# rubund/gnuais

Measured on AMD Instinct MI355X. Metric: Msamples/s demodulated (N-channel batch, full chain), higher is better.
Workload: dtype f32 FIR on int16 samples; u32 PLL/HDLC/CRC; 1 GPU; C3: 16384 ch x 48000 samples @48 kHz per GPU, full chain incl. HDLC/CRC-16; channels_per_gpu=16384, samples_per_channel=48000, parallelism=channels sharded over 1 GPU(s), one process per GPU, no collectives

## Files before the change

gnuais_amd/csrc/pll_common.h:

```cpp
#pragma once
#include <hip/hip_runtime.h>
#include <stdint.h>

#include "kernels.h"

namespace gnuais {

__device__ __forceinline__ uint32_t wave_max(uint32_t v)
{
#pragma unroll
    for (int o = 32; o; o >>= 1) {
        const uint32_t u = (uint32_t) __shfl_xor((int) v, o);
        v = u > v ? u : v;
    }
    return v;
}

constexpr int PLL_PACKW = PACK_STRIDE + 1;
constexpr int PLL_LUT_BYTES = 2048;

__device__ __forceinline__ void lds_flag_store(uint32_t *f, uint32_t v)
{
    asm volatile("" ::: "memory");
    __hip_atomic_store(f, v, __ATOMIC_RELAXED, __HIP_MEMORY_SCOPE_WORKGROUP);
    asm volatile("" ::: "memory");
}
__device__ __forceinline__ uint32_t lds_flag_load(uint32_t *f)
{
    asm volatile("" ::: "memory");
    const uint32_t v = __hip_atomic_load(f, __ATOMIC_RELAXED, __HIP_MEMORY_SCOPE_WORKGROUP);
    asm volatile("" ::: "memory");
    return v;
}

__host__ __device__ inline int n_seg_cap(int L)
{
    return (((L + 31) >> 5) + SEG_WORDS - 1) / SEG_WORDS;
}

__device__ __forceinline__ void pll_fill_lut(uint64_t *lut, int tid, int n_threads)
{
    for (int v = tid; v < 256; v += n_threads) {
        uint64_t e = 0;
        int n = 0;
        for (int b = 7; b >= 0; --b)
            if (v & (1 << b)) e |= (uint64_t) (7 - b) << (8 * n++);
        lut[v] = e;
    }
}

}
```

gnuais_amd/csrc/pll_h3.hip:

```cpp
#include <hip/hip_runtime.h>
#include <stdint.h>

#include <algorithm>
#include "kernels.h"
#include "pll_common.h"

namespace gnuais {

constexpr int H3_BLK = 128;
constexpr int H3_WORDS = H3_BLK / 32;
constexpr int H3_STRIP = H3_BLK + 12;
constexpr int H3_SEG_BLKS = SEG_LEN / H3_BLK;
constexpr int H3_NH = 3;
constexpr int H3_SLOTS = 2 * H3_NH;
constexpr int H3_NPACK = 4;
constexpr int H3_OFF_CNT = 64 * H3_STRIP, H3_OFF_NG = H3_OFF_CNT + 256;
constexpr int H3_SLOT_BYTES = H3_OFF_NG + 64;
constexpr int H3_FLAG_WORDS = 32 + 2 * 64 + 4 * 64;
constexpr int H3_NEED_LDS = PLL_LUT_BYTES + H3_SLOTS * H3_SLOT_BYTES + H3_NPACK * PLL_PACKW * 64 * 4 + H3_FLAG_WORDS * 4;
static_assert((H3_STRIP / 4) % 2 == 1 && H3_STRIP % 4 == 0, "odd dword stride: lanes hit different banks");
static_assert(SEG_LEN % H3_BLK == 0 && H3_NEED_LDS <= PLL_LDS_BYTES, "segments are whole blocks; the stage's LDS share");

enum { F_RDONE = 1, F_SEGPUB = 2, F_WRITTEN = 3, F_LAST = 4, F_SCAN = 8  };


__device__ __forceinline__ void h3_expand_block(const uint32_t (&S)[H3_WORDS], uint32_t &prev, int nv, uint8_t *lds,
                                                uint8_t *slot, const uint64_t *lut, int lane)
{
    uint32_t cur = (uint32_t) (slot - lds) + (uint32_t) (lane * H3_STRIP);
    const uint32_t cur0 = cur;
#pragma unroll
    for (int w = 0; w < H3_WORDS; ++w) {
        const int k = nv - 32 * w;
        uint32_t d = S[w] ^ ((S[w] >> 1) | (prev << 31));
        if (k <= 0) {
            d = 0;
        } else if (k < 32) {
            d &= ~0u << (32 - k);
            prev = (S[w] >> (32 - k)) & 1u;
        } else {
            prev = S[w] & 1u;
        }
        uint64_t ent[4];
#pragma unroll
        for (int y = 0; y < 4; ++y)
            ent[y] = lut[(d >> (24 - 8 * y)) & 0xffu];
#pragma unroll
        for (int y = 0; y < 4; ++y) {
            const uint32_t base = 0x01010101u * (uint32_t) (32 * w + 8 * y);
            const uint64_t e = ent[y] + (((uint64_t) base << 32) | base);
            asm volatile("ds_write_b64 %0, %1" :: "v"(cur), "v"(e) : "memory");
            cur += (uint32_t) __popc((d >> (24 - 8 * y)) & 0xffu);
        }
    }
    const uint32_t cnt = cur - cur0;
    reinterpret_cast<uint32_t *>(slot + H3_OFF_CNT)[lane] = cnt;
    const uint32_t ng = wave_max((cnt + 3u) >> 2);
    if (lane == 0) reinterpret_cast<uint32_t *>(slot + H3_OFF_NG)[0] = ng;
}

#define H3_STEP(k, E, kk)                                                                 \
    "v_cmpx_lt_i32 vcc, " #kk ", %[rem]\n\t"                                              \
    "v_mul_u32_u24_sdwa %[T], %[K8], %[" #E "] dst_sel:DWORD dst_unused:UNUSED_PAD src0_sel:DWORD src1_sel:BYTE_" #k "\n\t" \
    "v_add_u32 %[U], %[X], %[T]\n\t"                                                      \
    "v_bfe_i32 %[um], %[U], 23, 1\n\t"                                                    \
    "v_xad_u32 %[X], %[Q], %[um], %[X]\n\t"                                               \
    "v_lshlrev_b32_sdwa %[T], %[U], %[one] dst_sel:DWORD dst_unused:UNUSED_PAD src0_sel:BYTE_3 src1_sel:DWORD\n\t" \
    "v_xor_b32 %[M], %[M], %[T]\n\t"

__device__ __forceinline__ uint32_t h3_rows(uint32_t &X, uint32_t cnt, uint32_t ad, uint32_t ng, uint32_t Q, uint32_t K8)
{
    uint32_t U, um, T, E, F, G, H, M = 0, one = 1;
    int32_t rem = (int32_t) cnt;
    uint32_t np = (ng + 1u) >> 1;
    unsigned long long sv;
    asm volatile(
        "s_mov_b64 %[sv], exec\n\t"
        "ds_read_b32 %[E], %[ad]\n\t"
        "ds_read_b32 %[F], %[ad] offset:4\n\t"
        "1:\n\t"
        "ds_read_b32 %[G], %[ad] offset:8\n\t"
        "ds_read_b32 %[H], %[ad] offset:12\n\t"
        "s_waitcnt lgkmcnt(2)\n\t"
        "v_or_b32 %[X], 0xff, %[X]\n\t"
        H3_STEP(0, E, 0) H3_STEP(1, E, 1) H3_STEP(2, E, 2) H3_STEP(3, E, 3)
        "v_or_b32 %[X], 0xff, %[X]\n\t"
        H3_STEP(0, F, 4) H3_STEP(1, F, 5) H3_STEP(2, F, 6) H3_STEP(3, F, 7)
        "s_sub_u32 %[np], %[np], 1\n\t"
        "s_cmp_eq_u32 %[np], 0\n\t"
        "s_cbranch_scc1 2f\n\t"
        "ds_read_b32 %[E], %[ad] offset:16\n\t"
        "ds_read_b32 %[F], %[ad] offset:20\n\t"
        "s_waitcnt lgkmcnt(2)\n\t"
        "v_or_b32 %[X], 0xff, %[X]\n\t"
        H3_STEP(0, G, 8) H3_STEP(1, G, 9) H3_STEP(2, G, 10) H3_STEP(3, G, 11)
        "v_or_b32 %[X], 0xff, %[X]\n\t"
        H3_STEP(0, H, 12) H3_STEP(1, H, 13) H3_STEP(2, H, 14) H3_STEP(3, H, 15)
        "v_add_u32 %[ad], 16, %[ad]\n\t"
        "v_subrev_u32 %[rem], 16, %[rem]\n\t"
        "s_sub_u32 %[np], %[np], 1\n\t"
        "s_cmp_lg_u32 %[np], 0\n\t"
        "s_cbranch_scc1 1b\n\t"
        "2:\n\t"
        "s_mov_b64 exec, %[sv]\n\t"
        "s_waitcnt lgkmcnt(0)\n\t"
        : [X] "+v"(X), [U] "=&v"(U), [um] "=&v"(um), [T] "=&v"(T), [E] "=&v"(E), [F] "=&v"(F), [G] "=&v"(G), [H] "=&v"(H),
          [M] "+v"(M), [ad] "+v"(ad), [rem] "+v"(rem), [np] "+s"(np), [sv] "=&s"(sv)
        : [Q] "s"(Q), [K8] "v"(K8), [one] "v"(one)
        : "vcc", "scc", "memory");
    return M;
}

__device__ __forceinline__ uint32_t h3_write_pack(uint32_t *pk, uint32_t nb, uint32_t par, bool live,
                                                  uint32_t *__restrict__ dst, uint32_t *__restrict__ dcnt)
{
    uint32_t pd = 0;
#pragma unroll 1
    for (int g = 0; g < PACK_STRIDE / 4; ++g) {
        uint32_t o[4];
#pragma unroll
        for (int j = 0; j < 4; ++j) {
            const int w = 4 * g + j;
            const uint32_t tg = pk[w * 64];
            pk[w * 64] = 0;
            const int k = (int) nb - 32 * w;
            o[j] = ~tg & (k >= 32 ? ~0u : k > 0 ? (1u << k) - 1u : 0u);
            if (k >= 0 && k < 32) pd = (tg >> k) & 1u;
        }
        if (g == 0 && nb) o[0] ^= par;
        if (live) reinterpret_cast<uint4 *>(dst)[g] = make_uint4(o[0], o[1], o[2], o[3]);
    }
    if (live) *dcnt = nb;
    return nb ? pd : (par ^ pd);
}

__global__ __launch_bounds__(64 * (1 + H3_NH)) __attribute__((amdgpu_waves_per_eu(4, 8))) void pll_h3_kernel(
    const uint4 *__restrict__ sgn4, uint32_t *__restrict__ pllst, uint32_t *__restrict__ prevst,
    uint32_t *__restrict__ lastbit, uint32_t *__restrict__ segbits, uint32_t *__restrict__ segcnt,
    uint32_t *__restrict__ watchdog, int N, int L, int n_seg_alloc, uint32_t pllinc)
{
    extern __shared__ uint8_t lds[];
    uint64_t *lut = reinterpret_cast<uint64_t *>(lds);
    uint8_t *slots = lds + PLL_LUT_BYTES;
    uint32_t *pack = reinterpret_cast<uint32_t *>(slots + H3_SLOTS * H3_SLOT_BYTES);
    uint32_t *flag = pack + H3_NPACK * PLL_PACKW * 64;
    uint32_t *sign0 = flag + 32, *sign1 = flag + 32 + 64;
    uint32_t *nbuf = flag + 32 + 128;
    const int lane = threadIdx.x & 63, role = threadIdx.x >> 6;
    const int cg = blockIdx.x * 64 + lane;
    const int c = cg < N ? cg : N - 1;
    const bool live = cg < N;
    const int n_seg = n_seg_cap(L);
    const int n_blk = (L + H3_BLK - 1) / H3_BLK;
    if (threadIdx.x < 32) flag[threadIdx.x] = (threadIdx.x >= F_SCAN && threadIdx.x < F_SCAN + H3_NH) ? threadIdx.x - F_SCAN : 0u;
    if (role == 0) sign0[lane] = prevst[c] & 1u;
    pll_fill_lut(lut, (int) threadIdx.x, 64 * (1 + H3_NH));
    for (int q = threadIdx.x; q < H3_NPACK * PLL_PACKW * 64; q += 64 * (1 + H3_NH)) pack[q] = 0;
    __syncthreads();
    const unsigned long long t_start = wall_clock64();
    auto expired = [=]() {
        if (wall_clock64() - t_start <= 20000000ull) return false;
        if (lane == 0) atomicOr(watchdog, 1u);
        return true;
    };
#define peek(f) __builtin_amdgcn_readfirstlane((int) lds_flag_load(flag + (f)))
    __builtin_amdgcn_s_setprio(3);

    if (role >= 1) {
        const int h = role - 1;
        const uint4 *__restrict__ src = sgn4 + c;
        uint32_t par = h == 0 ? (lastbit[c] ^ sign0[lane]) & 1u : 0u;
        int wseg = 0;
#define H3_LOAD_BLOCK(b)                                   \
    do {                                                                                                        \
        const int bb = (b) < n_blk ? (b) : 0;                                                                   \
        q = src[(size_t) bb * (size_t) N];                                                                      \
        pw = reinterpret_cast<const uint32_t *>(src + (size_t) (bb > 0 ? bb - 1 : 0) * (size_t) N)[3];          \
    } while (0)
        uint4 q;
        uint32_t pw;
        H3_LOAD_BLOCK(h);
        bool dead = false;
        for (int bs = h; !dead; bs += H3_NH) {
            if (bs >= n_blk && !(h == 0 && wseg < n_seg)) break;
            if (h == 0) {
                while (wseg < n_seg && peek(F_SEGPUB) >= wseg + 1) {
                    uint32_t *pk = pack + (wseg & (H3_NPACK - 1)) * PLL_PACKW * 64 + lane;
                    const uint32_t nb = nbuf[(wseg & 3) * 64 + lane];
                    par = h3_write_pack(pk, nb, par, live, segbits + ((size_t) cg * n_seg_alloc + wseg) * PACK_STRIDE,
                                        segcnt + (size_t) cg * n_seg_alloc + wseg);
                    lds_flag_store(flag + F_WRITTEN, (uint32_t) (++wseg));
                }
                if (bs >= n_blk) {
                    if (expired()) dead = true;
                    __builtin_amdgcn_s_sleep(4);
                    continue;
                }
            }
            while (peek(F_RDONE) < bs - (H3_SLOTS - 1) && !dead) {
                if (expired()) dead = true;
                __builtin_amdgcn_s_sleep(8);
            }
            if (dead) break;
            {
                uint32_t S[H3_WORDS] = {q.x, q.y, q.z, q.w};
                uint32_t prev = bs == 0 ? sign0[lane] : (pw & 1u);
                H3_LOAD_BLOCK(bs + H3_NH);
                h3_expand_block(S, prev, L - bs * H3_BLK, lds, slots + (bs % H3_SLOTS) * H3_SLOT_BYTES, lut, lane);
                lds_flag_store(flag + F_SCAN + h, (uint32_t) (bs + H3_NH));
                if (bs == n_blk - 1) {
                    sign1[lane] = prev;
                    lds_flag_store(flag + F_LAST, 1u);
                    if (live) prevst[cg] = prev;
                }
            }
        }
        if (h == 0) {
            while (lds_flag_load(flag + F_LAST) == 0 && !dead)
                if (expired()) dead = true;
            if (live && !dead) {
                for (int s = n_seg; s < n_seg_alloc; ++s) segcnt[(size_t) cg * n_seg_alloc + s] = 0;
                lastbit[cg] = (sign1[lane] ^ par) & 1u;
            }
        }
        return;
    }

    uint32_t X = ((pllst[c] & 0xffffu) << 8) | 0xffu;
    const uint32_t Q = (uint32_t) __builtin_amdgcn_readfirstlane((int) ((pllinc / 16u) << 8));
    const uint32_t K8 = pllinc << 8;
    bool dead = false;
    for (int s = 0; s < n_seg && !dead; ++s) {
        while (peek(F_WRITTEN) < s - (H3_NPACK - 1) && !dead) {
            if (expired()) dead = true;
            __builtin_amdgcn_s_sleep(2);
        }
        uint32_t segbase = 0;
        uint32_t *pk = pack + (s & (H3_NPACK - 1)) * PLL_PACKW * 64 + lane;
        const int b1 = (s + 1) * H3_SEG_BLKS < n_blk ? (s + 1) * H3_SEG_BLKS : n_blk;
        for (int b = s * H3_SEG_BLKS; b < b1 && !dead; ++b) {
            const uint8_t *slot = slots + (b % H3_SLOTS) * H3_SLOT_BYTES;
            uint32_t cnt, ng;
            for (;;) {
                uint32_t f, g;
                asm volatile("ds_read_b32 %0, %3\n\tds_read_b32 %1, %4\n\tds_read_b32 %2, %5\n\ts_waitcnt lgkmcnt(0)"
                             : "=&v"(f), "=&v"(cnt), "=&v"(g)
                             : "v"((uint32_t) (reinterpret_cast<uint8_t *>(flag + F_SCAN + b % H3_NH) - lds)),
                               "v"((uint32_t) (slot + H3_OFF_CNT - lds) + (uint32_t) lane * 4u),
                               "v"((uint32_t) (slot + H3_OFF_NG - lds))
                             : "memory");
                ng = (uint32_t) __builtin_amdgcn_readfirstlane((int) g);
                if (__builtin_amdgcn_readfirstlane((int) f) >= b + 1) break;
                if (expired()) { dead = true; break; }
                __builtin_amdgcn_s_sleep(1);
            }
            if (dead) break;
            segbase += X >> 24;
            X &= 0x00ffffffu;
            if (ng) {
                const uint32_t M = h3_rows(X, cnt, (uint32_t) (slot - lds) + (uint32_t) (lane * H3_STRIP), ng, Q, K8);
                lds_flag_store(flag + F_RDONE, (uint32_t) (b + 1));
                const uint32_t sh = segbase & 31u, w = segbase >> 5;
                atomicXor(pk + w * 64, M << sh);
                atomicXor(pk + w * 64 + 64, (M >> 1) >> (31u - sh));
            } else {
                lds_flag_store(flag + F_RDONE, (uint32_t) (b + 1));
            }
            const int blen = L - b * H3_BLK < H3_BLK ? L - b * H3_BLK : H3_BLK;
            X += (uint32_t) blen * K8;
        }
        if (dead) break;
        X |= 0xffu;
        nbuf[(s & 3) * 64 + lane] = segbase + (X >> 24);
        X = (X & 0x00ffff00u) | 0xffu;
        lds_flag_store(flag + F_SEGPUB, (uint32_t) (s + 1));
    }
    if (live && !dead) pllst[cg] = (X >> 8) & 0xffffu;
}

int pll_need_lds() { return H3_NEED_LDS; }

hipError_t pll_prepare_device()
{
    return hipFuncSetAttribute((const void *) pll_h3_kernel, hipFuncAttributeMaxDynamicSharedMemorySize, 160 * 1024);
}

int pll_form_of(const PllLaunch &a)
{
    if ((a.variant == 7 || (a.variant == 0 && a.N <= PLL_TP_MAX_CHANNELS)) && pll_tp_applicable(a)) return 7;
    return 8;
}

hipError_t launch_pll(const PllLaunch &a, hipStream_t stream)
{
    if (pll_form_of(a) == 7) return launch_pll_tp(a, stream);
    const int n_cu = a.n_cu > 0 ? a.n_cu : 256;
    const int groups = (a.N + 63) / 64, per_cu = (groups + n_cu - 1) / n_cu;
    const int lds = per_cu <= 1 ? std::max(H3_NEED_LDS, PLL_LDS_BYTES) : std::max(H3_NEED_LDS, (160 * 1024 / per_cu) & ~1023);
    if (lds > 160 * 1024) return hipErrorInvalidValue;
    hipLaunchKernelGGL(pll_h3_kernel, dim3(groups), dim3(64 * (1 + H3_NH)), lds, stream, (const uint4 *) a.sgn, a.pll, a.prev, a.lastbit,
                       a.segbits, a.segcnt, a.watchdog, a.N, a.L, a.n_seg, a.pllinc);
    return hipGetLastError();
}

}
```

Baseline: 1.646 million Msamples/s.

## Streamline H3 block expansion: alignbit transitions, SDWA LUT addressing, DPP max, pointer-stepped loads

Reworks the H3 transition-expansion producer. Full blocks now compute transitions with alignbit, and the partial-bit masking is kept only for the tail block. LUT addresses are formed directly with SDWA byte-select shifts, and the wave-wide max uses a DPP reduction that leaves the result in lane 63 instead of shuffle-xor. Block loads use incrementally stepped pointers with a readfirstlane'd scalar block index, and the row consumer handles odd group counts by entering the unrolled loop mid-way. The goal is fewer VALU and address instructions in the producer wave. The risks are reliance on the LUT sitting at LDS offset 0 and on the DPP row semantics being correct.

```diff
diff --git a/gnuais_amd/csrc/pll_common.h b/gnuais_amd/csrc/pll_common.h
--- a/gnuais_amd/csrc/pll_common.h
+++ b/gnuais_amd/csrc/pll_common.h
@@ -13,6 +13,20 @@
         const uint32_t u = (uint32_t) __shfl_xor((int) v, o);
         v = u > v ? u : v;
     }
+    return v;
+}
+
+__device__ __forceinline__ uint32_t wave_max_in_lane63(uint32_t v)
+{
+#define PLL_DPP_MAX(ctrl, rows) \
+    { const uint32_t u = (uint32_t) __builtin_amdgcn_update_dpp(0, (int) v, ctrl, rows, 0xf, false); v = u > v ? u : v; }
+    PLL_DPP_MAX(0x111, 0xf)
+    PLL_DPP_MAX(0x112, 0xf)
+    PLL_DPP_MAX(0x114, 0xf)
+    PLL_DPP_MAX(0x118, 0xf)
+    PLL_DPP_MAX(0x142, 0xa)
+    PLL_DPP_MAX(0x143, 0xc)
+#undef PLL_DPP_MAX
     return v;
 }
 
diff --git a/gnuais_amd/csrc/pll_h3.hip b/gnuais_amd/csrc/pll_h3.hip
--- a/gnuais_amd/csrc/pll_h3.hip
+++ b/gnuais_amd/csrc/pll_h3.hip
@@ -24,39 +24,62 @@
 enum { F_RDONE = 1, F_SEGPUB = 2, F_WRITTEN = 3, F_LAST = 4, F_SCAN = 8  };
 
 
-__device__ __forceinline__ void h3_expand_block(const uint32_t (&S)[H3_WORDS], uint32_t &prev, int nv, uint8_t *lds,
-                                                uint8_t *slot, const uint64_t *lut, int lane)
-{
-    uint32_t cur = (uint32_t) (slot - lds) + (uint32_t) (lane * H3_STRIP);
-    const uint32_t cur0 = cur;
+__device__ __forceinline__ void h3_expand_block(const uint32_t (&d)[H3_WORDS], uint8_t *lds, uint8_t *slot, int lane)
+{
+    const uint32_t cur0 = (uint32_t) (slot - lds) + (uint32_t) (lane * H3_STRIP);
+    uint32_t cur = cur0;
+    const uint32_t three = 3;
+#pragma unroll
+    for (int w = 0; w < H3_WORDS; ++w) {
+        uint32_t a[4], at[4];
+        asm("v_lshlrev_b32_sdwa %0, %1, %2 dst_sel:DWORD dst_unused:UNUSED_PAD src0_sel:DWORD src1_sel:BYTE_3" : "=v"(a[0]) : "v"(three), "v"(d[w]));
+        asm("v_lshlrev_b32_sdwa %0, %1, %2 dst_sel:DWORD dst_unused:UNUSED_PAD src0_sel:DWORD src1_sel:BYTE_2" : "=v"(a[1]) : "v"(three), "v"(d[w]));
+        asm("v_lshlrev_b32_sdwa %0, %1, %2 dst_sel:DWORD dst_unused:UNUSED_PAD src0_sel:DWORD src1_sel:BYTE_1" : "=v"(a[2]) : "v"(three), "v"(d[w]));
+        asm("v_lshlrev_b32_sdwa %0, %1, %2 dst_sel:DWORD dst_unused:UNUSED_PAD src0_sel:DWORD src1_sel:BYTE_0" : "=v"(a[3]) : "v"(three), "v"(d[w]));
+        uint64_t ent[4];
+#pragma unroll
+        for (int y = 0; y < 4; ++y)
+            ent[y] = *(const __attribute__((address_space(3))) uint64_t *) (uintptr_t) a[y];
+#pragma unroll
+        for (int y = 0; y < 4; ++y) {
+            at[y] = cur;
+            cur += (uint32_t) __popc(a[y]);
+        }
+#pragma unroll
+        for (int y = 0; y < 4; ++y) {
+            const uint32_t base = 0x01010101u * (uint32_t) (32 * w + 8 * y);
+            const uint64_t e = ent[y] + (((uint64_t) base << 32) | base);
+            asm volatile("ds_write_b64 %0, %1" :: "v"(at[y]), "v"(e) : "memory");
+        }
+    }
+    const uint32_t cnt = cur - cur0;
+    reinterpret_cast<uint32_t *>(slot + H3_OFF_CNT)[lane] = cnt;
+    const uint32_t ng = wave_max_in_lane63((cnt + 3u) >> 2);
+    if (lane == 63) reinterpret_cast<uint32_t *>(slot + H3_OFF_NG)[0] = ng;
+}
+
+__device__ __forceinline__ void h3_transitions_full(const uint32_t (&S)[H3_WORDS], uint32_t pw, uint32_t (&d)[H3_WORDS])
+{
+#pragma unroll
+    for (int w = 0; w < H3_WORDS; ++w)
+        d[w] = S[w] ^ __builtin_amdgcn_alignbit(w ? S[w - 1] : pw, S[w], 1);
+}
+
+__device__ __forceinline__ void h3_transitions_tail(const uint32_t (&S)[H3_WORDS], uint32_t &prev, int nv, uint32_t (&d)[H3_WORDS])
+{
 #pragma unroll
     for (int w = 0; w < H3_WORDS; ++w) {
         const int k = nv - 32 * w;
-        uint32_t d = S[w] ^ ((S[w] >> 1) | (prev << 31));
+        d[w] = S[w] ^ ((S[w] >> 1) | (prev << 31));
         if (k <= 0) {
-            d = 0;
+            d[w] = 0;
         } else if (k < 32) {
-            d &= ~0u << (32 - k);
+            d[w] &= ~0u << (32 - k);
             prev = (S[w] >> (32 - k)) & 1u;
         } else {
             prev = S[w] & 1u;
         }
-        uint64_t ent[4];
-#pragma unroll
-        for (int y = 0; y < 4; ++y)
-            ent[y] = lut[(d >> (24 - 8 * y)) & 0xffu];
-#pragma unroll
-        for (int y = 0; y < 4; ++y) {
-            const uint32_t base = 0x01010101u * (uint32_t) (32 * w + 8 * y);
-            const uint64_t e = ent[y] + (((uint64_t) base << 32) | base);
-            asm volatile("ds_write_b64 %0, %1" :: "v"(cur), "v"(e) : "memory");
-            cur += (uint32_t) __popc((d >> (24 - 8 * y)) & 0xffu);
-        }
-    }
-    const uint32_t cnt = cur - cur0;
-    reinterpret_cast<uint32_t *>(slot + H3_OFF_CNT)[lane] = cnt;
-    const uint32_t ng = wave_max((cnt + 3u) >> 2);
-    if (lane == 0) reinterpret_cast<uint32_t *>(slot + H3_OFF_NG)[0] = ng;
+    }
 }
 
 #define H3_STEP(k, E, kk)                                                                 \
@@ -76,6 +99,16 @@
     unsigned long long sv;
     asm volatile(
         "s_mov_b64 %[sv], exec\n\t"
+        "s_bitcmp0_b32 %[ng], 0\n\t"
+        "s_cbranch_scc1 0f\n\t"
+        "v_subrev_u32 %[ad], 4, %[ad]\n\t"
+        "v_add_u32 %[rem], 4, %[rem]\n\t"
+        "ds_read_b32 %[F], %[ad] offset:4\n\t"
+        "ds_read_b32 %[G], %[ad] offset:8\n\t"
+        "ds_read_b32 %[H], %[ad] offset:12\n\t"
+        "s_waitcnt lgkmcnt(2)\n\t"
+        "s_branch 3f\n\t"
+        "0:\n\t"
         "ds_read_b32 %[E], %[ad]\n\t"
         "ds_read_b32 %[F], %[ad] offset:4\n\t"
         "1:\n\t"
@@ -84,6 +117,7 @@
         "s_waitcnt lgkmcnt(2)\n\t"
         "v_or_b32 %[X], 0xff, %[X]\n\t"
         H3_STEP(0, E, 0) H3_STEP(1, E, 1) H3_STEP(2, E, 2) H3_STEP(3, E, 3)
+        "3:\n\t"
         "v_or_b32 %[X], 0xff, %[X]\n\t"
         H3_STEP(0, F, 4) H3_STEP(1, F, 5) H3_STEP(2, F, 6) H3_STEP(3, F, 7)
         "s_sub_u32 %[np], %[np], 1\n\t"
@@ -106,7 +140,7 @@
         "s_waitcnt lgkmcnt(0)\n\t"
         : [X] "+v"(X), [U] "=&v"(U), [um] "=&v"(um), [T] "=&v"(T), [E] "=&v"(E), [F] "=&v"(F), [G] "=&v"(G), [H] "=&v"(H),
           [M] "+v"(M), [ad] "+v"(ad), [rem] "+v"(rem), [np] "+s"(np), [sv] "=&s"(sv)
-        : [Q] "s"(Q), [K8] "v"(K8), [one] "v"(one)
+        : [Q] "s"(Q), [K8] "v"(K8), [one] "v"(one), [ng] "s"(ng)
         : "vcc", "scc", "memory");
     return M;
 }
@@ -168,20 +202,17 @@
 
     if (role >= 1) {
         const int h = role - 1;
-        const uint4 *__restrict__ src = sgn4 + c;
         uint32_t par = h == 0 ? (lastbit[c] ^ sign0[lane]) & 1u : 0u;
         int wseg = 0;
-#define H3_LOAD_BLOCK(b)                                   \
-    do {                                                                                                        \
-        const int bb = (b) < n_blk ? (b) : 0;                                                                   \
-        q = src[(size_t) bb * (size_t) N];                                                                      \
-        pw = reinterpret_cast<const uint32_t *>(src + (size_t) (bb > 0 ? bb - 1 : 0) * (size_t) N)[3];          \
-    } while (0)
-        uint4 q;
-        uint32_t pw;
-        H3_LOAD_BLOCK(h);
+        const unsigned long long step1 = (unsigned long long) N * sizeof(uint4);
+        const int h0 = h < n_blk ? h : 0;
+        const uint4 *pq = sgn4 + (size_t) h0 * (size_t) N + c;
+        const uint32_t *ppw = reinterpret_cast<const uint32_t *>(sgn4 + (size_t) (h0 > 0 ? h0 - 1 : 0) * (size_t) N + c) + 3;
+        uint4 q = *pq;
+        uint32_t pw = *ppw;
         bool dead = false;
-        for (int bs = h; !dead; bs += H3_NH) {
+        for (int bv = h; !dead; bv += H3_NH) {
+            const int bs = __builtin_amdgcn_readfirstlane(bv);
             if (bs >= n_blk && !(h == 0 && wseg < n_seg)) break;
             if (h == 0) {
                 while (wseg < n_seg && peek(F_SEGPUB) >= wseg + 1) {
@@ -203,10 +234,23 @@
             }
             if (dead) break;
             {
-                uint32_t S[H3_WORDS] = {q.x, q.y, q.z, q.w};
-                uint32_t prev = bs == 0 ? sign0[lane] : (pw & 1u);
-                H3_LOAD_BLOCK(bs + H3_NH);
-                h3_expand_block(S, prev, L - bs * H3_BLK, lds, slots + (bs % H3_SLOTS) * H3_SLOT_BYTES, lut, lane);
+                const uint32_t S[H3_WORDS] = {q.x, q.y, q.z, q.w};
+                const uint32_t before = bs == 0 ? sign0[lane] : pw;
+                const bool more = bs + H3_NH < n_blk;
+                pq = reinterpret_cast<const uint4 *>(reinterpret_cast<const uint8_t *>(pq) + (more ? H3_NH * step1 : 0ull));
+                ppw = reinterpret_cast<const uint32_t *>(reinterpret_cast<const uint8_t *>(ppw) + (more ? (bs == 0 ? H3_NH - 1 : H3_NH) * step1 : 0ull));
+                q = *pq;
+                pw = *ppw;
+                uint8_t *slot = slots + (bs % H3_SLOTS) * H3_SLOT_BYTES;
+                const int nv = L - bs * H3_BLK;
+                uint32_t d[H3_WORDS], prev = S[H3_WORDS - 1] & 1u;
+                if (nv >= H3_BLK) {
+                    h3_transitions_full(S, before, d);
+                } else {
+                    prev = before & 1u;
+                    h3_transitions_tail(S, prev, nv, d);
+                }
+                h3_expand_block(d, lds, slot, lane);
                 lds_flag_store(flag + F_SCAN + h, (uint32_t) (bs + H3_NH));
                 if (bs == n_blk - 1) {
                     sign1[lane] = prev;
```

Measured after the change: 1.657 million Msamples/s, median of 6. Within noise of the previous version (+0.7%).
